# UPM-ROB-Lab/Vision-basedSensor

Measured on AMD Instinct MI355X. Metric: frames/sec (track->3D) at 1280x1024, 169 markers, higher is better.
Workload: dtype u8+f64; 1 GPU; BASELINE config 3/4: 4096 synthetic 1280x1024 gray uint8 frames per GPU (13x13 dots, seeded jitter+noise), resident in HBM; fused track->3D table + last-seen displacement; frames_per_gpu=4096, internal_batch=1536, pass_streams=2, markers=169, channels=1, world_size=1, backend=none (single process), distinct_devices=1, tracked_observations=692224, xyz_solved=692224, ncc_ambiguous_pixels=205, ncc_exact_pixels=11244250, ncc_counter_frames=839680

## Files before the change

### vision-basedsensor_amd/csrc/k_blur16.hip

```cpp
#include <algorithm>

#include "blur_common.h"

#define B16_NSW 7
#define B16_NS 8
#define B16_LD 4
template <bool SB> struct B16 {
    static constexpr int LEFT = SB ? 24 : 56;
    static constexpr int WIN = SB ? 64 : 128;
    static constexpr int NP = SB ? 11 : 15;
    static constexpr int ROWB = SB ? 208 : 272;
    static constexpr int DEPTH = SB ? 3 : 7;
    static constexpr int NVF = SB ? 8 : 12;
    static constexpr int WG_LEFT = SB ? 32 : 64;
};

template <bool U8OUT, bool SB, bool SHIFT>
__global__ __launch_bounds__(64 * (B16_NSW + 1), 4) void k_blur16(const u8* __restrict__ gray, int64_t gstride_n, int gstride_row,
                                                   const uint4* __restrict__ hfrag, const uint4* __restrict__ vfrag,
                                                   u64* __restrict__ bits, u8* __restrict__ area_u8,
                                                   u32* __restrict__ fstat, int H, int W, int WW, int tiles_per_seg,
                                                   int k3, int k8, int span_i, int nframes, int gx, int gy, int dbg_drop) {
    typedef B16<SB> G;
    constexpr int B16_LEFT_ = G::LEFT, B16_NP = G::NP, B16_ROWB = G::ROWB, DEPTH = G::DEPTH;
    __shared__ uint4 vf[G::NVF * 64];
    __shared__ __align__(16) u8 stg[B16_NS][16 * G::ROWB];
    __shared__ u32 staged;
    __shared__ u32 done[B16_NS];
    const int tid = threadIdx.x, lane = tid & 63;
    const int wave = __builtin_amdgcn_readfirstlane(tid >> 6);
    const int g = lane >> 4, q = lane & 15;
    int n, bx, by;
    if (nframes) {
        const int b = blockIdx.x, per = gx * gy, j = b >> 3;
        n = 8 * (j / per) + (b & 7);
        const int w = j % per;
        bx = w % gx; by = w / gx;
        if (n >= nframes) return;
    } else { n = blockIdx.z; bx = blockIdx.x; by = blockIdx.y; }
    const int tilesY = (H + 15) / 16;
    const int tile0 = by * tiles_per_seg;
    const int ntiles = min(tiles_per_seg, tilesY - tile0);
    if (ntiles <= 0) return;
    for (int i = tid; i < G::NVF * 64; i += 64 * (B16_NSW + 1)) vf[i] = vfrag[i];
    const bool is_loader = wave == B16_NSW;
    const int strip = bx * B16_NSW + wave, xw = 16 * strip;
    const int Y0 = tile0 * 16, nsteps = ntiles + DEPTH;
    const bool live = !is_loader && xw < W;
    if (!is_loader && !live && xw < 64 * WW)
        for (int y = Y0 + lane; y < min(Y0 + 16 * ntiles, H); y += 64)
            reinterpret_cast<unsigned short*>(bits)[((int64_t)n * H + y) * WW * 4 + strip] = 0;
    const int L0 = min(max(xw - B16_LEFT_, 0), W - G::WIN);
    const bool edge = !SB && L0 != xw - B16_LEFT_;
    v4i lp, lq, sq, sp = {0, 0, 0, 0};
    {
        const uint4* hf = hfrag + (size_t)min(strip, (W + 15) / 16 - 1) * 4 * 64 + lane;
        const uint4 b = hf[64], c = hf[128];
        lq = v4i{(int)b.x, (int)b.y, (int)b.z, (int)b.w};
        sq = v4i{(int)c.x, (int)c.y, (int)c.z, (int)c.w};
        lp = v4i{0, 0, 0, 0};
        if (!SB) { const uint4 a = hf[0]; lp = v4i{(int)a.x, (int)a.y, (int)a.z, (int)a.w}; }
        if (edge) { const uint4 d = hf[192]; sp = v4i{(int)d.x, (int)d.y, (int)d.z, (int)d.w}; }
    }
    const u8* gf = gray + (int64_t)n * gstride_n;
    const int X0 = min(max(16 * B16_NSW * bx - G::WG_LEFT, 0), W - 16 * B16_NP);
    const int XB = SHIFT ? (X0 & ~7) : X0;
    typedef u32 u32x4 __attribute__((ext_vector_type(4)));
    __builtin_amdgcn_s_waitcnt(0x0F70);
    if (tid < B16_NS) done[tid] = 0;
    if (tid == B16_NS) staged = 0;
    __syncthreads();

    if (is_loader) {
        int prow[4];
        bool pval[4];
        u32 poff[4];
        u8* pdst[4];
#pragma unroll
        for (int k = 0; k < 4; ++k) {
            const int id = 64 * k + lane;
            pval[k] = id < 16 * B16_NP;
            prow[k] = pval[k] ? id / B16_NP : 0;
            const int pc = pval[k] ? id - B16_NP * prow[k] : 0;
            poff[k] = (u32)(__mul24(prow[k], gstride_row) + X0 + 16 * pc);
            pdst[k] = &stg[0][0] + B16_ROWB * prow[k] + 16 * pc;
        }
        u32x4 R[B16_LD][4];
#pragma unroll
        for (int j = 0; j < B16_LD; ++j)
#pragma unroll
            for (int k = 0; k < 4; ++k) R[j][k] = u32x4{0, 0, 0, 0};
        auto row_of = [&](int t, int r) { return reflect101(Y0 - B16_LEFT_ + 16 * t + r, H); };
        auto issue = [&](int t, u32x4 (&Rt)[4]) {
            const int yt = Y0 - B16_LEFT_ + 16 * t;
            u32 o[4];
            if (yt >= 0 && yt + 15 < H) {
#pragma unroll
                for (int k = 0; k < 4; ++k) o[k] = (u32)(yt * gstride_row) + poff[k];
            } else {
#pragma unroll
                for (int k = 0; k < 4; ++k) o[k] = (u32)(__mul24(row_of(t, prow[k]) - prow[k], gstride_row)) + poff[k];
            }
            asm volatile("global_load_dwordx4 %0, %4, %8\n\tglobal_load_dwordx4 %1, %5, %8\n\t"
                         "global_load_dwordx4 %2, %6, %8\n\tglobal_load_dwordx4 %3, %7, %8"
                         : "=&v"(Rt[0]), "=&v"(Rt[1]), "=&v"(Rt[2]), "=&v"(Rt[3])
                         : "v"(o[0]), "v"(o[1]), "v"(o[2]), "v"(o[3]), "s"(gf) : "memory");
        };
#pragma unroll
        for (int j = 0; j < B16_LD; ++j) issue(j, R[j]);
        int slot = 0, gen = 0;
        bool lost = false;
        for (int t0 = 0; t0 < nsteps; t0 += B16_LD) {
#pragma unroll
            for (int j = 0; j < B16_LD; ++j) {
                const int t = t0 + j;
                if (t >= nsteps) break;
                if (gen > 0) {
                    const u32 want = (u32)(B16_NSW * gen);
                    bool ok = false;
                    for (int spin = 0; spin < (lost ? 1 : (1 << 20)); ++spin) {
                        const u32 have = __hip_atomic_load(&done[slot], __ATOMIC_ACQUIRE, __HIP_MEMORY_SCOPE_WORKGROUP);
                        if (__builtin_amdgcn_readfirstlane(have) >= want) { ok = true; break; }
                        __builtin_amdgcn_s_sleep(1);
                    }
                    if (!ok && !lost) { lost = true; if (lane == 0) atomicMin((int*)&fstat[n * 8 + 2], VBS_EINTERNAL); }
                }
                static_assert(B16_LD == 4, "the wait below leaves the B16_LD - 1 younger tiles' loads outstanding");
                asm volatile("s_waitcnt vmcnt(12)" : "+v"(R[j][0]), "+v"(R[j][1]), "+v"(R[j][2]), "+v"(R[j][3]) :: "memory");
                const int sb = slot * (16 * B16_ROWB);
#pragma unroll
                for (int k = 0; k < 4; ++k) {
                    u8* dst = pdst[k] + sb;
                    const uint4 v = make_uint4(R[j][k].x ^ 0x80808080u, R[j][k].y ^ 0x80808080u,
                                               R[j][k].z ^ 0x80808080u, R[j][k].w ^ 0x80808080u);
                    if (!SHIFT || X0 == XB) {
                        if (pval[k]) *reinterpret_cast<uint4*>(__builtin_assume_aligned(dst, 16)) = v;
                    } else if (pval[k]) {
                        u32* d32 = reinterpret_cast<u32*>(dst + (X0 - XB));
                        d32[0] = v.x; d32[1] = v.y; d32[2] = v.z; d32[3] = v.w;
                    }
                }
#ifdef VBS_DEBUG_KNOBS
                if (!(dbg_drop > 0 && t == dbg_drop - 1 && bx == 0 && by == 0))
#endif
                if (lane == 0) __hip_atomic_fetch_add(&staged, 1u, __ATOMIC_RELEASE, __HIP_MEMORY_SCOPE_WORKGROUP);
                issue(t + B16_LD, R[j]);
                if (++slot == B16_NS) { slot = 0; ++gen; }
            }
        }
#pragma unroll
        for (int j = 0; j < B16_LD; ++j)
            asm volatile("s_waitcnt vmcnt(0)" : "+v"(R[j][0]), "+v"(R[j][1]), "+v"(R[j][2]), "+v"(R[j][3]) :: "memory");
        return;
    }

    const u8* const rP = &stg[0][0] + B16_ROWB * q + (L0 - XB) + 16 * g + (g >= 2 ? 64 : 0);
    const u8* const rQ = &stg[0][0] + B16_ROWB * q + (L0 - XB) + (SB ? 0 : 32) + 16 * g;
    int rslot = 0;
    u32 rt = 0, known = 0;
    bool lost = false;
    auto read_ops = [&](uint4& p, uint4& qq) {
        if (rt >= known) {
            for (int spin = 0; spin < (lost ? 1 : (1 << 20)); ++spin) {
                known = (u32)__builtin_amdgcn_readfirstlane((int)__hip_atomic_load(&staged, __ATOMIC_ACQUIRE, __HIP_MEMORY_SCOPE_WORKGROUP));
                if (rt < known) break;
                __builtin_amdgcn_s_sleep(1);
            }
            if (rt >= known && !lost) { lost = true; if (lane == 0) atomicMin((int*)&fstat[n * 8 + 2], VBS_EINTERNAL); }
        }
        const uint2* b = reinterpret_cast<const uint2*>(rQ + rslot * (16 * B16_ROWB));
        const uint2 b0 = b[0], b1 = b[1];
        qq = make_uint4(b0.x, b0.y, b1.x, b1.y);
        if (!SB) {
            const uint2* a = reinterpret_cast<const uint2*>(rP + rslot * (16 * B16_ROWB));
            const uint2 a0 = a[0], a1 = a[1];
            p = make_uint4(a0.x, a0.y, a1.x, a1.y);
        }
        ++rt;
        if (++rslot == B16_NS) rslot = 0;
    };
    int dslot = 0;
    auto tick_done = [&]() {
        if (lane == 0) __hip_atomic_fetch_add(&done[dslot], 1u, __ATOMIC_RELEASE, __HIP_MEMORY_SCOPE_WORKGROUP);
        if (++dslot == B16_NS) dslot = 0;
    };
    v4i LhA = {0, 0, 0, 0}, LhB = {0, 0, 0, 0}, LlA = {0, 0, 0, 0}, LlB = {0, 0, 0, 0};
    v4i S4h = {0, 0, 0, 0}, S4l = {0, 0, 0, 0};
    int Sdh[4] = {0, 0, 0, 0}, Sdl[4] = {0, 0, 0, 0};
    const u32 span = (u32)span_i;
    const u32 m16 = xw + 16 <= W ? 0xFFFFu : (live ? ((1u << (W - xw)) - 1u) : 0u);
    const u64 colmask = (u64)m16 * 0x0001000100010001ull;
    unsigned short* mb16 = reinterpret_cast<unsigned short*>(bits) + (int64_t)n * H * WW * 4 + strip;
    const u32 sel1 = 0u - ((u32)lane & 1u), sel2 = 0u - (((u32)lane >> 1) & 1u);
    u32 total = 0, pp[4] = {0, 0, 0, 0};
    auto flush_rows = [&](int tg) {
#pragma unroll
        for (int k = 0; k < 8; ++k) {
            const int y = Y0 + 16 * (tg + k - DEPTH) + lane;
            if (live && lane < 16 && tg + k >= DEPTH && tg + k < nsteps && y < H)
                mb16[(u32)__mul24(y, 4 * WW)] = (unsigned short)(pp[k >> 1] >> (16 * (k & 1)));
        }
    };
    auto finish_tile = [&](const v4i& d8, const v4i& d3, int yo, int u) {
            u64 pw[4];
#pragma unroll
            for (int i = 0; i < 4; ++i) {
                const u32 dg = (((u32)d8[i] >> 16) - ((u32)d3[i] >> 16)) & 255u;
                pw[i] = __ballot(dg <= span) & colmask;
            }
            if (yo + 15 >= H) {
#pragma unroll
                for (int i = 0; i < 4; ++i) pw[i] &= __ballot(yo + 4 * g + i < H);
            }
            total += (u32)(__popcll(pw[0]) + __popcll(pw[1]) + __popcll(pw[2]) + __popcll(pw[3]));
            if (U8OUT) {
#pragma unroll
                for (int i = 0; i < 4; ++i) {
                    const int y = yo + 4 * g + i, x = xw + q;
                    if (y < H && x < W) area_u8[((int64_t)n * H + y) * W + x] = (u8)(((pw[i] >> lane) & 1ull) ? 255 : 0);
                }
            }
            {
                const u32 x01l = (u32)pw[0] ^ (u32)pw[1], x01h = (u32)(pw[0] >> 32) ^ (u32)(pw[1] >> 32);
                const u32 x23l = (u32)pw[2] ^ (u32)pw[3], x23h = (u32)(pw[2] >> 32) ^ (u32)(pw[3] >> 32);
                const u32 t0l = (x01l & sel1) ^ (u32)pw[0], t0h = (x01h & sel1) ^ (u32)(pw[0] >> 32);
                const u32 t1l = (x23l & sel1) ^ (u32)pw[2], t1h = (x23h & sel1) ^ (u32)(pw[2] >> 32);
                const u32 vl = ((t0l ^ t1l) & sel2) ^ t0l, vh = ((t0h ^ t1h) & sel2) ^ t0h;
                const u32 piece = ((lane & 8 ? vh : vl) >> (16 * ((lane >> 2) & 1))) & 0xFFFFu;
                pp[u >> 1] = (u & 1) ? (pp[u >> 1] | (piece << 16)) : piece;
            }
    };
    uint4 aP_ = make_uint4(0, 0, 0, 0), aQ_;
    read_ops(aP_, aQ_);
    for (int t0 = 0; t0 < nsteps; t0 += 8) {
#pragma unroll
        for (int u = 0; u < 8; ++u) {
            const int t = t0 + u;
            if (t >= nsteps) break;
            const v4i aP = v4i{(int)aP_.x, (int)aP_.y, (int)aP_.z, (int)aP_.w}, aQ = v4i{(int)aQ_.x, (int)aQ_.y, (int)aQ_.z, (int)aQ_.w};
            if (!SB) {
            const uint4 fa_ = vf[u * 64 + lane], fb_ = vf[((u + 4) & 7) * 64 + lane], fs_ = vf[(8 + (u & 3)) * 64 + lane];
            v4i accL = {0, 0, 0, 0}, accS = {0, 0, 0, 0};
            accL = __builtin_amdgcn_mfma_i32_16x16x64_i8(aP, lp, accL, 0, 0, 0);
            accS = __builtin_amdgcn_mfma_i32_16x16x64_i8(aQ, sq, accS, 0, 0, 0);
            accL = __builtin_amdgcn_mfma_i32_16x16x64_i8(aQ, lq, accL, 0, 0, 0);
            if (edge) accS = __builtin_amdgcn_mfma_i32_16x16x64_i8(aP, sp, accS, 0, 0, 0);
            tick_done();
            if (t + 1 < nsteps) read_ops(aP_, aQ_);
            {
                int hi, lo;
                pack16(accL, hi, lo);
                if (u < 4) { LhA[u & 3] = hi; LlA[u & 3] = lo; } else { LhB[u & 3] = hi; LlB[u & 3] = lo; }
                pack16(accS, hi, lo);
                Sdh[u & 3] = hi; Sdl[u & 3] = lo;
                S4h[(u + 2) & 3] = Sdh[(u + 2) & 3];
                S4l[(u + 2) & 3] = Sdl[(u + 2) & 3];
            }
            if (t >= DEPTH) {
            const v4i fa = v4i{(int)fa_.x, (int)fa_.y, (int)fa_.z, (int)fa_.w}, fb = v4i{(int)fb_.x, (int)fb_.y, (int)fb_.z, (int)fb_.w};
            const v4i fs = v4i{(int)fs_.x, (int)fs_.y, (int)fs_.z, (int)fs_.w};
            v4i d8 = {0, 0, 0, 0}, d3 = {0, 0, 0, 0};
            d8 = __builtin_amdgcn_mfma_i32_16x16x64_i8(fa, LhA, d8, 0, 0, 0);
            d3 = __builtin_amdgcn_mfma_i32_16x16x64_i8(fs, S4h, d3, 0, 0, 0);
            d8 = __builtin_amdgcn_mfma_i32_16x16x64_i8(fb, LhB, d8, 0, 0, 0);
#pragma unroll
            for (int i = 0; i < 4; ++i) d3[i] = (d3[i] << 8) + k3;
            d3 = __builtin_amdgcn_mfma_i32_16x16x64_i8(fs, S4l, d3, 0, 0, 0);
#pragma unroll
            for (int i = 0; i < 4; ++i) d8[i] = (d8[i] << 8) + k8;
            d8 = __builtin_amdgcn_mfma_i32_16x16x64_i8(fa, LlA, d8, 0, 0, 0);
            d8 = __builtin_amdgcn_mfma_i32_16x16x64_i8(fb, LlB, d8, 0, 0, 0);
            finish_tile(d8, d3, Y0 + 16 * (t - DEPTH), u);
            }
            } else {
            const uint4 fa_ = vf[(u & 3) * 64 + lane], fs_ = vf[(4 + (u & 3)) * 64 + lane];
            v4i accL = {0, 0, 0, 0}, accS = {0, 0, 0, 0};
            accL = __builtin_amdgcn_mfma_i32_16x16x64_i8(aQ, lq, accL, 0, 0, 0);
            accS = __builtin_amdgcn_mfma_i32_16x16x64_i8(aQ, sq, accS, 0, 0, 0);
            tick_done();
            if (t + 1 < nsteps) read_ops(aP_, aQ_);
            {
                int hi, lo;
                pack16(accL, hi, lo);
                LhA[u & 3] = hi; LlA[u & 3] = lo;
                pack16(accS, hi, lo);
                S4h[u & 3] = hi; S4l[u & 3] = lo;
            }
            if (t >= DEPTH) {
            const v4i fa = v4i{(int)fa_.x, (int)fa_.y, (int)fa_.z, (int)fa_.w}, fs = v4i{(int)fs_.x, (int)fs_.y, (int)fs_.z, (int)fs_.w};
            v4i d8 = {0, 0, 0, 0}, d3 = {0, 0, 0, 0};
            d8 = __builtin_amdgcn_mfma_i32_16x16x64_i8(fa, LhA, d8, 0, 0, 0);
            d3 = __builtin_amdgcn_mfma_i32_16x16x64_i8(fs, S4h, d3, 0, 0, 0);
#pragma unroll
            for (int i = 0; i < 4; ++i) d8[i] = (d8[i] << 8) + k8;
#pragma unroll
            for (int i = 0; i < 4; ++i) d3[i] = (d3[i] << 8) + k3;
            d8 = __builtin_amdgcn_mfma_i32_16x16x64_i8(fa, LlA, d8, 0, 0, 0);
            d3 = __builtin_amdgcn_mfma_i32_16x16x64_i8(fs, S4l, d3, 0, 0, 0);
            finish_tile(d8, d3, Y0 + 16 * (t - DEPTH), u);
            }
            }
            if (u == 7) flush_rows(t0);
        }
    }
    if (nsteps & 7) flush_rows(nsteps & ~7);
    if (live && lane == 0 && total) atomicAdd(&fstat[n * 8 + 0], total);
}

void blur16_fragments(const std::vector<int>& taps_s, const std::vector<int>& taps_l, int W, bool small, std::vector<u32>* hfrag,
                      std::vector<u32>* vfrag) {
    const int nstrips = (W + 15) / 16;
    const int LEFT = small ? B16<true>::LEFT : B16<false>::LEFT, WIN = small ? B16<true>::WIN : B16<false>::WIN;
    auto refl = [&](int i) { if (i < 0) i = -i; if (i >= W) i = 2 * (W - 1) - i; return std::min(std::max(i, 0), W - 1); };
    hfrag->assign((size_t)nstrips * 4 * 64 * 4, 0);
    for (int s = 0; s < nstrips; ++s) {
        const int xw = 16 * s, L0 = std::min(std::max(xw - LEFT, 0), W - WIN);
        for (int f = 0; f < 4; ++f) {
            if (small && (f == 0 || f == 3)) continue;
            const std::vector<int>& taps = f < 2 ? taps_l : taps_s;
            const int R = (int)taps.size() / 2;
            const bool useP = (f == 0 || f == 3);
            for (int lane = 0; lane < 64; ++lane) {
                const int g = lane >> 4, x = std::min(xw + (lane & 15), W - 1);
                for (int e = 0; e < 16; ++e) {
                    const int k = 16 * g + e, w = small ? k : (useP ? (k < 32 ? k : k + 64) : 32 + k), xin = L0 + w;
                    int c = 0;
                    for (int j = 0; j <= 2 * R; ++j) if (refl(x + j - R) == xin) c += taps[j];
                    (*hfrag)[(((size_t)s * 4 + f) * 64 + lane) * 4 + (e >> 2)] |= (u32)(c & 255) << (8 * (e & 3));
                }
            }
        }
    }
    const int nv = small ? 8 : 12, nl = small ? 4 : 8;
    vfrag->assign((size_t)nv * 64 * 4, 0);
    for (int v = 0; v < nv; ++v) {
        const std::vector<int>& taps = v < nl ? taps_l : taps_s;
        const int R = (int)taps.size() / 2;
        for (int lane = 0; lane < 64; ++lane) {
            const int g = lane >> 4, m = lane & 15;
            for (int e = 0; e < 16; ++e) {
                const int pos = e >> 2, i = e & 3;
                int a;
                if (small) a = (((v < nl ? v : v - nl) - pos) % 4 + 4) % 4;
                else a = v < 8 ? ((v - pos) % 8 + 8) % 8 : 2 + (((v - 8) - pos - 2) % 4 + 4) % 4;
                const int k = R + LEFT - 16 * a + 4 * g + i - m;
                const u32 c = (k >= 0 && k <= 2 * R) ? (u32)taps[k] : 0u;
                (*vfrag)[((size_t)v * 64 + lane) * 4 + (e >> 2)] |= c << (8 * (e & 3));
            }
        }
    }
}

static bool blur16_takes(const vbs_handle* h, const u8* gray, int64_t gstride_n, int64_t gstride_row) {
    const int minw = 16 * (h->bp.small ? B16<true>::NP : B16<false>::NP);
    return h->blur_impl == 0 && h->blur16_h && h->W >= minw && (h->W & 3) == 0 && h->H >= 64 &&
           (reinterpret_cast<uintptr_t>(gray) & 3) == 0 && (gstride_n & 3) == 0 && (gstride_row & 3) == 0 &&
           gstride_row >= h->W && gstride_row < (1 << 23) && (int64_t)h->H * gstride_row < (1ll << 31);
}

static void launch_blur16(vbs_handle* h, Workspace& w, const u8* gray, int64_t gstride_n, int64_t gstride_row, int nb,
                          u8* area_u8, hipStream_t s) {
    const int k3 = 256 * (128 + 32768) + 32768, k8 = k3 + (15 - h->bp.thresh) * 65536;
    const int gx16 = (4 * h->WW + B16_NSW - 1) / B16_NSW, tiles16 = (h->H + 15) / 16;
    int nseg = std::min(tiles16 / 8, std::max(1, (2048 + gx16 * nb - 1) / (gx16 * nb)));
    nseg = std::max(nseg, 1);
    if (VBS_KNOB("VBS_BLUR16_NSEG")) nseg = VBS_KNOB("VBS_BLUR16_NSEG");
    const int tps = (tiles16 + nseg - 1) / nseg;
    nseg = (tiles16 + tps - 1) / tps;
    const int xcd = nb >= 32 ? nb : 0;
    dim3 grid16 = xcd ? dim3((unsigned)((nb + 7) / 8 * 8 * gx16 * nseg)) : dim3(gx16, nseg, nb);
#define B16_GO(U8, SB_, SH_)                                                                                                  \
    VBS_LAUNCH(h, s, "k_blur16", (k_blur16<U8, SB_, SH_>), grid16, dim3(64 * (B16_NSW + 1)), 0, s, gray, gstride_n,              \
               (int)gstride_row, h->blur16_h, h->blur16_v, w.area_bits, area_u8, w.fstat, h->H, h->W, h->WW, tps, k3, k8,     \
               h->bp.hi - h->bp.thresh, xcd, gx16, nseg, VBS_KNOB("VBS_BLUR16_DROP"))
#define B16_GO2(U8, SB_) do { if (h->W & 7) B16_GO(U8, SB_, true); else B16_GO(U8, SB_, false); } while (0)
    if (h->bp.small) { if (area_u8) B16_GO2(true, true); else B16_GO2(false, true); }
    else { if (area_u8) B16_GO2(true, false); else B16_GO2(false, false); }
#undef B16_GO2
#undef B16_GO
}

void launch_blur(vbs_handle* h, Workspace& w, const u8* gray, int64_t gstride_n, int64_t gstride_row, int nb,
                 u8* area_u8, hipStream_t s) {
    if (blur16_takes(h, gray, gstride_n, gstride_row)) launch_blur16(h, w, gray, gstride_n, gstride_row, nb, area_u8, s);
    else launch_blur_mfma(h, w, gray, gstride_n, gstride_row, nb, area_u8, s);
}
```

Before: 294,100 frames/s.

## Transpose vertical MFMA output so each lane owns a row nibble, dropping ballots

The A and B operands of the vertical-pass MFMAs are swapped so that the output tile comes out transposed, with each lane holding 4 horizontal pixels of one row. The threshold mask is then built as a per-lane nibble instead of four wave-wide ballots plus an XOR bit-transpose. Packed row bits are gathered with permlane32/permlane16 swaps at flush time, bottom-edge and column masking move into the flush, and the popcount total is reduced with a shuffle once at the end. The u8 area output becomes one 32-bit store per lane, so a 4-byte alignment check on area_u8 is added, and the new lane-to-row mapping must match the previous bit layout exactly.

```diff
diff --git a/vision-basedsensor_amd/csrc/k_blur16.hip b/vision-basedsensor_amd/csrc/k_blur16.hip
--- a/vision-basedsensor_amd/csrc/k_blur16.hip
+++ b/vision-basedsensor_amd/csrc/k_blur16.hip
@@ -189,46 +189,49 @@
     int Sdh[4] = {0, 0, 0, 0}, Sdl[4] = {0, 0, 0, 0};
     const u32 span = (u32)span_i;
     const u32 m16 = xw + 16 <= W ? 0xFFFFu : (live ? ((1u << (W - xw)) - 1u) : 0u);
-    const u64 colmask = (u64)m16 * 0x0001000100010001ull;
     unsigned short* mb16 = reinterpret_cast<unsigned short*>(bits) + (int64_t)n * H * WW * 4 + strip;
-    const u32 sel1 = 0u - ((u32)lane & 1u), sel2 = 0u - (((u32)lane >> 1) & 1u);
+    const u32 lmask = (((m16 >> (4 * g)) & 15u) * 0x00010001u) << (4 * g);
+    const u32 sh_even = (u32)(4 * g), sh_odd = (u32)(4 * g + 16);
     u32 total = 0, pp[4] = {0, 0, 0, 0};
     auto flush_rows = [&](int tg) {
-#pragma unroll
-        for (int k = 0; k < 8; ++k) {
-            const int y = Y0 + 16 * (tg + k - DEPTH) + lane;
-            if (live && lane < 16 && tg + k >= DEPTH && tg + k < nsteps && y < H)
-                mb16[(u32)__mul24(y, 4 * WW)] = (unsigned short)(pp[k >> 1] >> (16 * (k & 1)));
-        }
+        if (Y0 + 16 * (tg + 8 - DEPTH) > H) {
+#pragma unroll
+            for (int k = 0; k < 8; ++k)
+                if (Y0 + 16 * (tg + k - DEPTH) + q >= H) pp[k >> 1] &= (k & 1) ? 0x0000FFFFu : 0xFFFF0000u;
+        }
+#pragma unroll
+        for (int k = 0; k < 4; ++k) {
+            pp[k] &= lmask;
+            total += (u32)__popc(pp[k]);
+        }
+        const auto s01 = __builtin_amdgcn_permlane32_swap(pp[0], pp[1], false, false);
+        const auto s23 = __builtin_amdgcn_permlane32_swap(pp[2], pp[3], false, false);
+        const auto s = __builtin_amdgcn_permlane16_swap(s01[0] | s01[1], s23[0] | s23[1], false, false);
+        const u32 w = s[0] | s[1];
+        const int k0 = tg + 2 * (((g & 1) << 1) | (g >> 1));
+#pragma unroll
+        for (int hh = 0; hh < 2; ++hh) {
+            const int y = Y0 + 16 * (k0 + hh - DEPTH) + q;
+            if (live && k0 + hh >= DEPTH && k0 + hh < nsteps && y < H)
+                mb16[(u32)__mul24(y, 4 * WW)] = (unsigned short)(w >> (16 * hh));
+        }
+#pragma unroll
+        for (int k = 0; k < 4; ++k) pp[k] = 0;
     };
     auto finish_tile = [&](const v4i& d8, const v4i& d3, int yo, int u) {
-            u64 pw[4];
+            u32 nib = 0;
 #pragma unroll
             for (int i = 0; i < 4; ++i) {
                 const u32 dg = (((u32)d8[i] >> 16) - ((u32)d3[i] >> 16)) & 255u;
-                pw[i] = __ballot(dg <= span) & colmask;
-            }
-            if (yo + 15 >= H) {
-#pragma unroll
-                for (int i = 0; i < 4; ++i) pw[i] &= __ballot(yo + 4 * g + i < H);
-            }
-            total += (u32)(__popcll(pw[0]) + __popcll(pw[1]) + __popcll(pw[2]) + __popcll(pw[3]));
+                nib |= dg <= span ? (1u << i) : 0u;
+            }
             if (U8OUT) {
-#pragma unroll
-                for (int i = 0; i < 4; ++i) {
-                    const int y = yo + 4 * g + i, x = xw + q;
-                    if (y < H && x < W) area_u8[((int64_t)n * H + y) * W + x] = (u8)(((pw[i] >> lane) & 1ull) ? 255 : 0);
-                }
-            }
-            {
-                const u32 x01l = (u32)pw[0] ^ (u32)pw[1], x01h = (u32)(pw[0] >> 32) ^ (u32)(pw[1] >> 32);
-                const u32 x23l = (u32)pw[2] ^ (u32)pw[3], x23h = (u32)(pw[2] >> 32) ^ (u32)(pw[3] >> 32);
-                const u32 t0l = (x01l & sel1) ^ (u32)pw[0], t0h = (x01h & sel1) ^ (u32)(pw[0] >> 32);
-                const u32 t1l = (x23l & sel1) ^ (u32)pw[2], t1h = (x23h & sel1) ^ (u32)(pw[2] >> 32);
-                const u32 vl = ((t0l ^ t1l) & sel2) ^ t0l, vh = ((t0h ^ t1h) & sel2) ^ t0h;
-                const u32 piece = ((lane & 8 ? vh : vl) >> (16 * ((lane >> 2) & 1))) & 0xFFFFu;
-                pp[u >> 1] = (u & 1) ? (pp[u >> 1] | (piece << 16)) : piece;
-            }
+                const int y = yo + q, x = xw + 4 * g;
+                if (y < H && x < W)
+                    *reinterpret_cast<u32*>(area_u8 + ((int64_t)n * H + y) * W + x) =
+                        ((nib & 1u) ? 0xFFu : 0u) | ((nib & 2u) ? 0xFF00u : 0u) | ((nib & 4u) ? 0xFF0000u : 0u) | ((nib & 8u) ? 0xFF000000u : 0u);
+            }
+            pp[u >> 1] |= nib << ((u & 1) ? sh_odd : sh_even);
     };
     uint4 aP_ = make_uint4(0, 0, 0, 0), aQ_;
     read_ops(aP_, aQ_);
@@ -260,16 +263,16 @@
             const v4i fa = v4i{(int)fa_.x, (int)fa_.y, (int)fa_.z, (int)fa_.w}, fb = v4i{(int)fb_.x, (int)fb_.y, (int)fb_.z, (int)fb_.w};
             const v4i fs = v4i{(int)fs_.x, (int)fs_.y, (int)fs_.z, (int)fs_.w};
             v4i d8 = {0, 0, 0, 0}, d3 = {0, 0, 0, 0};
-            d8 = __builtin_amdgcn_mfma_i32_16x16x64_i8(fa, LhA, d8, 0, 0, 0);
-            d3 = __builtin_amdgcn_mfma_i32_16x16x64_i8(fs, S4h, d3, 0, 0, 0);
-            d8 = __builtin_amdgcn_mfma_i32_16x16x64_i8(fb, LhB, d8, 0, 0, 0);
+            d8 = __builtin_amdgcn_mfma_i32_16x16x64_i8(LhA, fa, d8, 0, 0, 0);
+            d3 = __builtin_amdgcn_mfma_i32_16x16x64_i8(S4h, fs, d3, 0, 0, 0);
+            d8 = __builtin_amdgcn_mfma_i32_16x16x64_i8(LhB, fb, d8, 0, 0, 0);
 #pragma unroll
             for (int i = 0; i < 4; ++i) d3[i] = (d3[i] << 8) + k3;
-            d3 = __builtin_amdgcn_mfma_i32_16x16x64_i8(fs, S4l, d3, 0, 0, 0);
+            d3 = __builtin_amdgcn_mfma_i32_16x16x64_i8(S4l, fs, d3, 0, 0, 0);
 #pragma unroll
             for (int i = 0; i < 4; ++i) d8[i] = (d8[i] << 8) + k8;
-            d8 = __builtin_amdgcn_mfma_i32_16x16x64_i8(fa, LlA, d8, 0, 0, 0);
-            d8 = __builtin_amdgcn_mfma_i32_16x16x64_i8(fb, LlB, d8, 0, 0, 0);
+            d8 = __builtin_amdgcn_mfma_i32_16x16x64_i8(LlA, fa, d8, 0, 0, 0);
+            d8 = __builtin_amdgcn_mfma_i32_16x16x64_i8(LlB, fb, d8, 0, 0, 0);
             finish_tile(d8, d3, Y0 + 16 * (t - DEPTH), u);
             }
             } else {
@@ -289,14 +292,14 @@
             if (t >= DEPTH) {
             const v4i fa = v4i{(int)fa_.x, (int)fa_.y, (int)fa_.z, (int)fa_.w}, fs = v4i{(int)fs_.x, (int)fs_.y, (int)fs_.z, (int)fs_.w};
             v4i d8 = {0, 0, 0, 0}, d3 = {0, 0, 0, 0};
-            d8 = __builtin_amdgcn_mfma_i32_16x16x64_i8(fa, LhA, d8, 0, 0, 0);
-            d3 = __builtin_amdgcn_mfma_i32_16x16x64_i8(fs, S4h, d3, 0, 0, 0);
+            d8 = __builtin_amdgcn_mfma_i32_16x16x64_i8(LhA, fa, d8, 0, 0, 0);
+            d3 = __builtin_amdgcn_mfma_i32_16x16x64_i8(S4h, fs, d3, 0, 0, 0);
 #pragma unroll
             for (int i = 0; i < 4; ++i) d8[i] = (d8[i] << 8) + k8;
 #pragma unroll
             for (int i = 0; i < 4; ++i) d3[i] = (d3[i] << 8) + k3;
-            d8 = __builtin_amdgcn_mfma_i32_16x16x64_i8(fa, LlA, d8, 0, 0, 0);
-            d3 = __builtin_amdgcn_mfma_i32_16x16x64_i8(fs, S4l, d3, 0, 0, 0);
+            d8 = __builtin_amdgcn_mfma_i32_16x16x64_i8(LlA, fa, d8, 0, 0, 0);
+            d3 = __builtin_amdgcn_mfma_i32_16x16x64_i8(S4l, fs, d3, 0, 0, 0);
             finish_tile(d8, d3, Y0 + 16 * (t - DEPTH), u);
             }
             }
@@ -304,6 +307,8 @@
         }
     }
     if (nsteps & 7) flush_rows(nsteps & ~7);
+#pragma unroll
+    for (int off = 32; off >= 1; off >>= 1) total += (u32)__shfl_xor((int)total, off);
     if (live && lane == 0 && total) atomicAdd(&fstat[n * 8 + 0], total);
 }
 
@@ -351,10 +356,11 @@
     }
 }
 
-static bool blur16_takes(const vbs_handle* h, const u8* gray, int64_t gstride_n, int64_t gstride_row) {
+static bool blur16_takes(const vbs_handle* h, const u8* gray, int64_t gstride_n, int64_t gstride_row, const u8* area_u8) {
     const int minw = 16 * (h->bp.small ? B16<true>::NP : B16<false>::NP);
     return h->blur_impl == 0 && h->blur16_h && h->W >= minw && (h->W & 3) == 0 && h->H >= 64 &&
-           (reinterpret_cast<uintptr_t>(gray) & 3) == 0 && (gstride_n & 3) == 0 && (gstride_row & 3) == 0 &&
+           (reinterpret_cast<uintptr_t>(gray) & 3) == 0 && (reinterpret_cast<uintptr_t>(area_u8) & 3) == 0 &&
+           (gstride_n & 3) == 0 && (gstride_row & 3) == 0 &&
            gstride_row >= h->W && gstride_row < (1 << 23) && (int64_t)h->H * gstride_row < (1ll << 31);
 }
 
@@ -382,6 +388,6 @@
 
 void launch_blur(vbs_handle* h, Workspace& w, const u8* gray, int64_t gstride_n, int64_t gstride_row, int nb,
                  u8* area_u8, hipStream_t s) {
-    if (blur16_takes(h, gray, gstride_n, gstride_row)) launch_blur16(h, w, gray, gstride_n, gstride_row, nb, area_u8, s);
+    if (blur16_takes(h, gray, gstride_n, gstride_row, area_u8)) launch_blur16(h, w, gray, gstride_n, gstride_row, nb, area_u8, s);
     else launch_blur_mfma(h, w, gray, gstride_n, gstride_row, nb, area_u8, s);
 }
```

Measured after the change: 294,900 frames/s (median of 5 runs). About the same (+0.3%).
